# votnhan/VN_celeb_face_recognition

Hardware: AMD Instinct MI355X
Metric: embeddings/sec @ bs=256 (InceptionResnetV1, 160x160) (higher is better)
Workload: dtype bf16

## Files before the change

vn_celeb_face_recognition_amd/csrc/aux_kernels.hip:

```cpp
#include <cstdlib>
#include <algorithm>
#include "kernels.h"
#include "storage_unit.h"

namespace vnf {

typedef __bf16 bf16x8_t __attribute__((ext_vector_type(8)));
typedef _Float16 f16x8_t __attribute__((ext_vector_type(8)));
typedef float f32x4_t __attribute__((ext_vector_type(4)));

template <typename T> __device__ __forceinline__ float to_f(T v) { return (float)v; }

template <typename TI, typename TO>
__global__ void pack_input_kernel(const TI* __restrict__ x, TO* __restrict__ y, int n, int hw) {
  const size_t total = (size_t)n * hw;
  for (size_t i = blockIdx.x * (size_t)blockDim.x + threadIdx.x; i < total; i += (size_t)gridDim.x * blockDim.x) {
    const size_t img = i / hw, p = i - img * hw;
    const TI* src = x + img * 3 * (size_t)hw + p;
    if constexpr (sizeof(TO) == sizeof(pf16) && __is_same(TO, pf16)) {
      const float v[8] = {to_f(src[0]), to_f(src[hw]), to_f(src[2 * (size_t)hw]), 0.f, 0.f, 0.f, 0.f, 0.f};
      Unit<pf16>::store(y + i * 8, v);
    } else {
      TO o[8];
      o[0] = (TO)to_f(src[0]);
      o[1] = (TO)to_f(src[hw]);
      o[2] = (TO)to_f(src[2 * (size_t)hw]);
#pragma unroll
      for (int c = 3; c < 8; ++c) o[c] = (TO)0.f;
      TO* dst = y + i * 8;
      if constexpr (sizeof(TO) == 2) {
        *reinterpret_cast<uint4*>(dst) = *reinterpret_cast<const uint4*>(o);
      } else {
        *reinterpret_cast<uint4*>(dst) = *reinterpret_cast<const uint4*>(o);
        *reinterpret_cast<uint4*>(dst + 4) = *reinterpret_cast<const uint4*>(o + 4);
      }
    }
  }
}

template <typename TI>
static hipError_t pack_dispatch_out(const void* x, void* out, int dtype, int n, int hw, hipStream_t s) {
  const size_t total = (size_t)n * hw;
  const int blocks = (int)((total + 255) / 256 < 4096 ? (total + 255) / 256 : 4096);
  if (blocks == 0) return hipSuccess;
  switch (dtype) {
    case BF16: hipLaunchKernelGGL((pack_input_kernel<TI, __bf16>), dim3(blocks), dim3(256), 0, s, (const TI*)x, (__bf16*)out, n, hw); break;
    case F16: hipLaunchKernelGGL((pack_input_kernel<TI, _Float16>), dim3(blocks), dim3(256), 0, s, (const TI*)x, (_Float16*)out, n, hw); break;
    case F32: hipLaunchKernelGGL((pack_input_kernel<TI, float>), dim3(blocks), dim3(256), 0, s, (const TI*)x, (float*)out, n, hw); break;
    case F16P: hipLaunchKernelGGL((pack_input_kernel<TI, pf16>), dim3(blocks), dim3(256), 0, s, (const TI*)x, (pf16*)out, n, hw); break;
    default: return hipErrorInvalidValue;
  }
  return hipGetLastError();
}

hipError_t launch_pack_input(const void* x, int x_dtype, void* out, int dtype, int n, int hw, hipStream_t s) {
  switch (x_dtype) {
    case F32: return pack_dispatch_out<float>(x, out, dtype, n, hw, s);
    case BF16: return pack_dispatch_out<__bf16>(x, out, dtype, n, hw, s);
    case F16: return pack_dispatch_out<_Float16>(x, out, dtype, n, hw, s);
  }
  return hipErrorInvalidValue;
}

typedef float f2_t __attribute__((ext_vector_type(2)));

template <typename TI, typename TO>
__global__ void __launch_bounds__(256) stem_conv1a_kernel(const TI* __restrict__ x, TO* __restrict__ y, int ldy, int n,
                                                          const float* __restrict__ wt) {
  constexpr int S = 160, SO = 79;
  const unsigned total = (unsigned)n * SO * SO;
  const unsigned i = blockIdx.x * blockDim.x + threadIdx.x;
  if (i >= total) return;
  const unsigned img = i / (SO * SO), p = i - img * (SO * SO);
  const int oy = (int)(p / SO), ox = (int)(p - (unsigned)oy * SO);
  const TI* src = x + (size_t)img * 3 * S * S + (size_t)(2 * oy) * S + 2 * ox;
  float in[27];
#pragma unroll
  for (int c = 0; c < 3; ++c)
#pragma unroll
    for (int kh = 0; kh < 3; ++kh)
#pragma unroll
      for (int kw = 0; kw < 3; ++kw) in[(c * 3 + kh) * 3 + kw] = to_f(src[(size_t)c * S * S + kh * S + kw]);
  f2_t acc[16];
#pragma unroll
  for (int j = 0; j < 16; ++j) acc[j] = f2_t{wt[27 * 32 + 2 * j], wt[27 * 32 + 2 * j + 1]};
#pragma unroll
  for (int k = 0; k < 27; ++k) {
    const f2_t v2 = {in[k], in[k]};
#pragma unroll
    for (int j = 0; j < 16; ++j) acc[j] = __builtin_elementwise_fma(v2, f2_t{wt[k * 32 + 2 * j], wt[k * 32 + 2 * j + 1]}, acc[j]);
  }
  if constexpr (__is_same(TO, pf16)) {
#pragma unroll
    for (int u = 0; u < 4; ++u) {
      float v[8];
#pragma unroll
      for (int j = 0; j < 4; ++j) { v[2 * j] = fmaxf(acc[4 * u + j][0], 0.f); v[2 * j + 1] = fmaxf(acc[4 * u + j][1], 0.f); }
      Unit<pf16>::store(y + (size_t)i * ldy + u * 8, v);
    }
  } else {
    TO o[32];
#pragma unroll
    for (int j = 0; j < 16; ++j) { o[2 * j] = (TO)fmaxf(acc[j][0], 0.f); o[2 * j + 1] = (TO)fmaxf(acc[j][1], 0.f); }
    uint4* dst = reinterpret_cast<uint4*>(y + (size_t)i * ldy);
#pragma unroll
    for (int q = 0; q < (int)(32 * sizeof(TO) / 16); ++q) dst[q] = reinterpret_cast<const uint4*>(o)[q];
  }
}

template <typename TI, typename TO>
__global__ void __launch_bounds__(256) stem_conv1a_mfma_kernel(const TI* __restrict__ x, TO* __restrict__ y, int ldy, int n,
                                                               const float* __restrict__ wt) {
  constexpr int S = 160, SO = 79, NPX = SO * SO, G = 4;
  const int lane = threadIdx.x & 63, col = lane & 15, g = lane >> 4;
  const unsigned total = (unsigned)n * NPX;
  const unsigned ngroups = (total + 15) / 16;
  const unsigned nwaves = gridDim.x * 4, w0 = blockIdx.x * 4 + (threadIdx.x >> 6);
  float wa[2][7], bias[2][4];
  int koff[7];
#pragma unroll
  for (int t = 0; t < 7; ++t) {
    const int k = 4 * t + g;
    wa[0][t] = k < 27 ? wt[k * 32 + col] : 0.f;
    wa[1][t] = k < 27 ? wt[k * 32 + 16 + col] : 0.f;
    koff[t] = k < 27 ? (k / 9) * S * S + ((k % 9) / 3) * S + k % 3 : 0;
  }
#pragma unroll
  for (int ct = 0; ct < 2; ++ct)
#pragma unroll
    for (int e = 0; e < 4; ++e) bias[ct][e] = wt[27 * 32 + 16 * ct + 4 * g + e];
  const int cst = (g & 1) * 16 + (g >> 1) * 8;
  for (unsigned gi = w0 * G; gi < ngroups; gi += nwaves * G) {
    float xb[G][7];
#pragma unroll
    for (int q = 0; q < G; ++q) {
      const unsigned i = min((gi + q) * 16 + col, total - 1);
      const unsigned img = i / NPX, p = i - img * NPX;
      const int oy = (int)(p / SO), ox = (int)(p - (unsigned)oy * SO);
      const TI* src = x + (size_t)img * 3 * S * S + (size_t)(2 * oy) * S + 2 * ox;
#pragma unroll
      for (int t = 0; t < 7; ++t) xb[q][t] = to_f(src[koff[t]]);
    }
#pragma unroll
    for (int q = 0; q < G; ++q) {
      typedef float f4 __attribute__((ext_vector_type(4)));
      f4 a0 = {bias[0][0], bias[0][1], bias[0][2], bias[0][3]}, a1 = {bias[1][0], bias[1][1], bias[1][2], bias[1][3]};
#pragma unroll
      for (int t = 0; t < 7; ++t) {
        a0 = __builtin_amdgcn_mfma_f32_16x16x4f32(wa[0][t], xb[q][t], a0, 0, 0, 0);
        a1 = __builtin_amdgcn_mfma_f32_16x16x4f32(wa[1][t], xb[q][t], a1, 0, 0, 0);
      }
      const unsigned i = (gi + q) * 16 + col;
      const bool ok = gi + q < ngroups && i < total;
      if constexpr (__is_same(TO, pf16)) {
        typedef _Float16 h4 __attribute__((ext_vector_type(4)));
        h4 h0, l0, h1, l1;
#pragma unroll
        for (int e = 0; e < 4; ++e) {
          const sf16 s0(fmaxf(a0[e], 0.f)), s1(fmaxf(a1[e], 0.f));
          h0[e] = s0.hi; l0[e] = s0.lo;
          h1[e] = s1.hi; l1[e] = s1.lo;
        }
        const uint2 ph0 = __builtin_bit_cast(uint2, h0), ph1 = __builtin_bit_cast(uint2, h1);
        const uint2 pl0 = __builtin_bit_cast(uint2, l0), pl1 = __builtin_bit_cast(uint2, l1);
        const auto hx = __builtin_amdgcn_permlane16_swap(ph0.x, ph1.x, false, false);
        const auto hy = __builtin_amdgcn_permlane16_swap(ph0.y, ph1.y, false, false);
        const auto lx = __builtin_amdgcn_permlane16_swap(pl0.x, pl1.x, false, false);
        const auto ly = __builtin_amdgcn_permlane16_swap(pl0.y, pl1.y, false, false);
        if (ok) {
          char* d = reinterpret_cast<char*>(y) + ((size_t)i * ldy + cst) * 4;
          *reinterpret_cast<uint4*>(d) = uint4{hx[0], hy[0], hx[1], hy[1]};
          *reinterpret_cast<uint4*>(d + 16) = uint4{lx[0], ly[0], lx[1], ly[1]};
        }
      } else {
        typedef TO t4 __attribute__((ext_vector_type(4)));
        t4 o0, o1;
#pragma unroll
        for (int e = 0; e < 4; ++e) { o0[e] = (TO)fmaxf(a0[e], 0.f); o1[e] = (TO)fmaxf(a1[e], 0.f); }
        const uint2 p0 = __builtin_bit_cast(uint2, o0), p1 = __builtin_bit_cast(uint2, o1);
        const auto sx = __builtin_amdgcn_permlane16_swap(p0.x, p1.x, false, false);
        const auto sy = __builtin_amdgcn_permlane16_swap(p0.y, p1.y, false, false);
        if (ok) *reinterpret_cast<uint4*>(y + (size_t)i * ldy + cst) = uint4{sx[0], sy[0], sx[1], sy[1]};
      }
    }
  }
}

template <typename TI>
static hipError_t stem_dispatch_out(const void* x, void* y, int ldy, int dtype, int n, const float* wt, bool mfma, hipStream_t s) {
  if (mfma && n > 0 && (dtype == BF16 || dtype == F16 || dtype == F16P)) {
    const unsigned ngroups = ((unsigned)n * 79 * 79 + 15) / 16;
    const int blocks = (int)((ngroups + 15) / 16 < 2048 ? (ngroups + 15) / 16 : 2048);
    if (dtype == BF16) hipLaunchKernelGGL((stem_conv1a_mfma_kernel<TI, __bf16>), dim3(blocks), dim3(256), 0, s, (const TI*)x, (__bf16*)y, ldy, n, wt);
    else if (dtype == F16) hipLaunchKernelGGL((stem_conv1a_mfma_kernel<TI, _Float16>), dim3(blocks), dim3(256), 0, s, (const TI*)x, (_Float16*)y, ldy, n, wt);
    else hipLaunchKernelGGL((stem_conv1a_mfma_kernel<TI, pf16>), dim3(blocks), dim3(256), 0, s, (const TI*)x, (pf16*)y, ldy, n, wt);
    return hipGetLastError();
  }
  const unsigned total = (unsigned)n * 79 * 79;
  const int blocks = (int)((total + 255) / 256);
  if (blocks == 0) return hipSuccess;
  switch (dtype) {
    case BF16: hipLaunchKernelGGL((stem_conv1a_kernel<TI, __bf16>), dim3(blocks), dim3(256), 0, s, (const TI*)x, (__bf16*)y, ldy, n, wt); break;
    case F16: hipLaunchKernelGGL((stem_conv1a_kernel<TI, _Float16>), dim3(blocks), dim3(256), 0, s, (const TI*)x, (_Float16*)y, ldy, n, wt); break;
    case F32: hipLaunchKernelGGL((stem_conv1a_kernel<TI, float>), dim3(blocks), dim3(256), 0, s, (const TI*)x, (float*)y, ldy, n, wt); break;
    case F16P: hipLaunchKernelGGL((stem_conv1a_kernel<TI, pf16>), dim3(blocks), dim3(256), 0, s, (const TI*)x, (pf16*)y, ldy, n, wt); break;
    default: return hipErrorInvalidValue;
  }
  return hipGetLastError();
}

hipError_t launch_stem_conv1a(const void* x, int x_dtype, void* y, int ldy, int dtype, int n, const float* wt, bool mfma,
                              hipStream_t s) {
  switch (x_dtype) {
    case F32: return stem_dispatch_out<float>(x, y, ldy, dtype, n, wt, mfma, s);
    case BF16: return stem_dispatch_out<__bf16>(x, y, ldy, dtype, n, wt, mfma, s);
    case F16: return stem_dispatch_out<_Float16>(x, y, ldy, dtype, n, wt, mfma, s);
  }
  return hipErrorInvalidValue;
}

template <typename T, int K, int PAD, bool INSIDE>
__global__ void maxpool_kernel(const T* __restrict__ x, int ldx, T* __restrict__ y, int ldy, int n, int H, int W, int C,
                               int Ho, int Wo) {
  typedef Unit<T> U;
  constexpr int N = U::N;
  constexpr bool kCeil = !INSIDE && PAD == 0;
  constexpr int TAPS = kCeil ? 1 : K;
  const int cc = C / N;
  const unsigned total = (unsigned)n * Ho * Wo * cc;
  for (unsigned i = blockIdx.x * blockDim.x + threadIdx.x; i < total; i += gridDim.x * blockDim.x) {
    const unsigned p = i / cc;
    const int c = (int)(i - p * cc) * N;
    const unsigned q = p / Wo;
    const int wo = (int)(p - q * Wo);
    const unsigned img = q / Ho;
    const int ho = (int)(q - img * Ho);
    float m[N];
#pragma unroll
    for (int e = 0; e < N; ++e) m[e] = -INFINITY;
    if constexpr (INSIDE && sizeof(typename U::Raw) == 16) {
      const T* xi = x + ((size_t)img * H * W + (size_t)(2 * ho) * W + 2 * wo) * ldx + c;
      typename U::Raw r[K * K];
#pragma unroll
      for (int dh = 0; dh < K; ++dh)
#pragma unroll
        for (int dw = 0; dw < K; ++dw) r[dh * K + dw] = U::raw(xi + (size_t)(dh * W + dw) * ldx);
#pragma unroll
      for (int t = 0; t < K * K; ++t)
#pragma unroll
// ... 402 lines not shown
```

vn_celeb_face_recognition_amd/csrc/conv_ws.hip:

```cpp
#include <type_traits>
#include <utility>

#include "conv_device.h"
#include "stamp.h"

namespace vnf {

template <typename T, int BM, int BN, int WM, int WN, int S, int LW, bool DBG = false>
__global__ __launch_bounds__((WM* WN + LW) * 64) void conv_igemm_ws_kernel(const KArgs a) {
  extern __shared__ __attribute__((aligned(16))) char smem[];
  constexpr int ES = (int)sizeof(T);
  constexpr int CH = 16 / ES, BKE = 128 / ES;
  constexpr int WTM = BM / WM, WTN = BN / WN, TM = WTM / 16, TN = WTN / 16;
  constexpr int NC = WM * WN, NT = (NC + LW) * 64;
  constexpr int PA = BM / 8, PB = BN / 8;
  constexpr int LA = PA / LW, LB = PB / LW;
  constexpr int STAGE = (BM + BN) * 128;
  constexpr int CST = BN + 4;
  constexpr int EPI_LDS = (BM * CST * 4 <= S * STAGE && (BM * (BN / 8)) / (NC * 64) <= 8) ? S * STAGE : (BM / WM) * CST * 4;
  constexpr int EPASS = (BM * CST * 4 <= EPI_LDS) ? 1 : WM;
  static_assert(S >= 3 && PA % LW == 0 && PB % LW == 0, "pieces divide over the loader waves");

  const int tid = threadIdx.x, lane = tid & 63;
  const int wave = __builtin_amdgcn_readfirstlane(tid >> 6);
// ... 494 lines not shown
          const uint2 ph0 = __builtin_bit_cast(uint2, h0), ph1 = __builtin_bit_cast(uint2, h1);
          const uint2 pl0 = __builtin_bit_cast(uint2, l0), pl1 = __builtin_bit_cast(uint2, l1);
          const auto hx = __builtin_amdgcn_permlane16_swap(ph0.x, ph1.x, false, false);
          const auto hy = __builtin_amdgcn_permlane16_swap(ph0.y, ph1.y, false, false);
          const auto lx = __builtin_amdgcn_permlane16_swap(pl0.x, pl1.x, false, false);
          const auto ly = __builtin_amdgcn_permlane16_swap(pl0.y, pl1.y, false, false);
          if (m < a.M && c < a.Cout) {
            char* d = dcol + (size_t)m * dld * ES;
            *reinterpret_cast<uint4*>(d) = uint4{hx[0], hy[0], hx[1], hy[1]};
            *reinterpret_cast<uint4*>(d + 16) = uint4{lx[0], ly[0], lx[1], ly[1]};
          }
        } else {
          tx4 o0, o1;
#pragma unroll
          for (int e = 0; e < 4; ++e) { o0[e] = (elem_t)v0[e]; o1[e] = (elem_t)v1[e]; }
          const uint2 p0 = __builtin_bit_cast(uint2, o0), p1 = __builtin_bit_cast(uint2, o1);
          const auto sx = __builtin_amdgcn_permlane16_swap(p0.x, p1.x, false, false);
          const auto sy = __builtin_amdgcn_permlane16_swap(p0.y, p1.y, false, false);
          if (m < a.M && c < a.Cout)
            *reinterpret_cast<uint4*>(dcol + (size_t)m * dld * ES) = uint4{sx[0], sy[0], sx[1], sy[1]};
        }
      }
    }
  }
}

struct WsCfg { int bm, bn, wm, wn, s, lw; };
static constexpr WsCfg kWs[] = {
    {256, 128, 2, 2, 3, 4}, {256, 128, 4, 1, 3, 4}, {128, 128, 2, 2, 3, 4}, {128, 128, 2, 2, 4, 4},
    {256, 64, 4, 1, 3, 4},  {128, 192, 2, 2, 3, 4}, {128, 256, 2, 2, 3, 4}, {128, 64, 2, 2, 4, 4},
    {256, 128, 2, 2, 3, 2}, {128, 128, 2, 2, 4, 2}, {128, 192, 2, 2, 3, 2}, {192, 128, 2, 2, 3, 4},
    {160, 256, 2, 2, 3, 4}, {160, 192, 2, 2, 3, 4},
    {64, 64, 2, 2, 4, 4},   {64, 128, 2, 2, 4, 4},  {32, 64, 2, 2, 6, 4},   {32, 128, 2, 2, 4, 4},  {64, 64, 2, 2, 8, 4},
};
constexpr int kNumWs = (int)(sizeof(kWs) / sizeof(kWs[0]));

int ws_num_cfgs() { return kNumWs; }
bool ws_cfg_tile(int wcfg, ConvTile& t) {
  if (wcfg < 0 || wcfg >= kNumWs) return false;
  t = ConvTile{2, kWs[wcfg].bm, kWs[wcfg].bn, kWs[wcfg].wm, kWs[wcfg].wn, kWs[wcfg].s};
  return true;
}

bool ws_cfg_ok(const ConvArgs& a, int wcfg) {
  if (wcfg < 0 || wcfg >= kNumWs) return false;
  const WsCfg& c = kWs[wcfg];
  if (a.Cout <= c.bn / 2) return false;
  if (((a.Cout + c.bn - 1) / c.bn) * c.bn > a.cout_pad) return false;
  if ((c.bn % 64) && a.Cout % c.bn) return false;
  const int lds = c.s * (c.bm + c.bn) * 128 + (a.Kpad / (128 / dtype_size(a.dtype))) * 8 * 16;
  return lds <= 160 * 1024;
}

template <typename T, int BM, int BN, int WM, int WN, int S, int LW>
static hipError_t launch_one_tile(const KArgs& k, hipStream_t s) {
  allow_dynamic_lds<conv_igemm_ws_kernel<T, BM, BN, WM, WN, S, LW>>(160 * 1024);
  KArgs kk = k;
  const int lds = S * (BM + BN) * 128 + k.nkt * 8 * 16;
  const int tiles_m = (k.M + BM - 1) / BM;
  kk.tiles_n = (k.Cout + BN - 1) / BN;
  kk.nblk = tiles_m * kk.tiles_n;
  hipLaunchKernelGGL((conv_igemm_ws_kernel<T, BM, BN, WM, WN, S, LW>), dim3(kk.nblk), dim3((WM * WN + LW) * 64), lds, s,
                     kk);
  return hipGetLastError();
}

// ... 106 lines not shown
```

vn_celeb_face_recognition_amd/csrc/engine.cpp:

```cpp
#include "engine.h"
#include "split_f16.h"

#include <cstdio>
#include <cstring>

namespace vnf {

static thread_local std::string g_err;
void set_error(const std::string& msg) { g_err = msg; }
int fail(int code, const std::string& msg) {
  g_err = msg;
  return code;
}
const char* last_error_cstr() { return g_err.c_str(); }

HandleBase::~HandleBase() {
  for (void* p : allocs) (void)hipFree(p);
}
void* HandleBase::dalloc(size_t bytes) {
  void* p = nullptr;
  if (bytes == 0) bytes = 16;
  hipError_t e = hipMalloc(&p, bytes);
  if (e != hipSuccess) {
    set_error(std::string("hipMalloc: ") + hipGetErrorString(e));
// ... 220 lines not shown
      const int nn = (i1 - n0) < step ? (i1 - n0) : step;
      for (int oi = g.first; oi < g.last; ++oi) {
        if (report) {
          hipEvent_t e0;
          VNF_HIP(hipEventCreate(&e0));
          VNF_HIP(hipEventRecord(e0, s));
          prof_ev.push_back(e0);
          prof_op.push_back(oi);
        }
        if (fused_at[oi] >= 0) {
          const FusedStack& f = fused[fused_at[oi]];
          const int rc = launch_fused(f, n0, nn, s);
          if (rc != VNF_OK) return rc;
          oi = f.end() - 1;
          continue;
        }
        const Op& op = ops[oi];
        const Buf* ib = op.src >= 0 ? &bufs[op.src] : nullptr;
        switch (op.kind) {
          case Op::PACK:
            if (ex.prep_src)
              VNF_HIP(launch_emotion_prep(ex.prep_src + (size_t)n0 * ex.prep_s * ex.prep_s * 3, nn, ex.prep_s, at(op.dst, n0), dtype, true, s));
            else
              VNF_HIP(launch_pack_input((const char*)x + n0 * x_image, x_dtype, at(op.dst, n0), dtype, nn, in_size * in_size, s));
            break;
          case Op::CONV: {
            const ConvLayer& L = convs[op.layer];
            hipError_t err = launch_conv(conv_args(L, n0, nn), s);
            if (err != hipSuccess) return fail(VNF_E_HIP, L.name + ": " + hipGetErrorString(err));
            break;
          }
          case Op::STEM1:
            VNF_HIP(launch_stem_conv1a((const char*)x + n0 * x_image, x_dtype, at(op.dst, n0), bufs[op.dst].C, dtype, nn, stem_wt,
                                       env.stem1a_mfma != 0, s));
            break;
          case Op::MAXPOOL:
            VNF_HIP(launch_maxpool(at(op.src, n0), ib->C, at(op.dst, n0, op.dst_coff), bufs[op.dst].C, dtype, nn, ib->H, ib->W, ib->C,
                                   op.window, s));
            break;
          case Op::AVGPOOL:
            VNF_HIP(launch_avgpool(at(op.src, n0), ib->C, at(op.dst, n0), dtype, nn, ib->H * ib->W, ib->C, s));
            break;
          case Op::L2NORM:
            VNF_HIP(launch_l2norm(emb_raw + (size_t)n0 * 512, out + (size_t)n0 * 512, nn, 512, s));
            break;
          case Op::DWCONV: {
            if (!f32_plan) return fail(VNF_E_INVALID, "depthwise conv: fp32 / split-f16 plans only");
            const DwLayer& d = dws[op.layer];
            const Buf& xb = bufs[d.x_buf];
            VNF_HIP(launch_dwconv3x3(at_f32(d.x_buf, n0), at_f32(d.o_buf, n0), nn, xb.H, xb.W, d.C, d.stride, d.w, d.bias, d.slope,
                                     dtype == F16X2, s));
            break;
          }
          case Op::RSTEM:
            if (!f32_plan || !x) return fail(VNF_E_INVALID, "retina stem: fp32 / split-f16 plans on caller frames only");
            VNF_HIP(launch_retina_stem((const uint8_t*)x + (size_t)n0 * op.frame_h * op.frame_w * 3, nn, op.frame_h, op.frame_w, rstem_wa,
                                       rstem_bias, 0.1f, at_f32(op.dst, n0), dtype == F16X2, s));
            break;
          case Op::DWPW: {
            if (!f32_plan) return fail(VNF_E_INVALID, "dw+pw: fp32 / split-f16 plans only");
            const DwPwLayer& d = dwpws[op.layer];
            const Buf& xb = bufs[d.x_buf];
            VNF_HIP(launch_dwpw(at_f32(d.x_buf, n0), at_f32(d.o_buf, n0), nn, xb.H, xb.W, d.cin, d.cout, d.stride, d.dw, d.dbias, d.slope,
                                d.pw, d.pbias, d.slope, dtype == F16X2, s));
            break;
          }
          case Op::UPADD: {
// ... 102 lines not shown
```

vn_celeb_face_recognition_amd/csrc/engine.h:

```cpp
#pragma once
#include <hip/hip_runtime.h>
#include <stdint.h>

#include <string>
#include <unordered_map>
#include <vector>

#include "../../include/vnface.h"
#include "kernels.h"

namespace vnf {

void set_error(const std::string& msg);
int fail(int code, const std::string& msg);
const char* last_error_cstr();

#define VNF_HIP(expr)                                                                         \
  do {                                                                                        \
    hipError_t _e = (expr);                                                                   \
    if (_e != hipSuccess)                                                                     \
      return ::vnf::fail(VNF_E_HIP, std::string(#expr) + ": " + hipGetErrorString(_e));       \
  } while (0)

enum class HandleKind { Encoder = 1, Mlp, Mtcnn, MlpTrainer, Retina, HeadTrainer, ConvProbe };
// ... 97 lines not shown
  float slope = 0.f;
  std::string name;
};

struct SeLayer {
  std::string name;
  int C, part_buf;
  float *w1 = nullptr, *b1 = nullptr, *w2 = nullptr, *b2 = nullptr;
  float slope_se = 0.f, slope_out = 0.f;
};

struct Group { int first, last, chunk; };

struct FusedStack {
  enum class Kind { StemMid, Block35, Block17 } kind = Kind::Block17;
  int first = 0, last = 0;
  int in_buf = -1, out_buf = -1;
  int nblocks = 0;
  int conv0 = 0;
  void* wstream = nullptr;
  float* bias = nullptr;
  void* wtail = nullptr;
  bool active = false;
  bool stack = false;
  double macs_alg = 0;
  int ext_last = 0, ext_conv = -1, ext_out_buf = -1;
  bool ext = false;
  int end() const { return ext ? ext_last : last; }
};

struct Tap { int buf, coff, C; };

struct EncoderEnv {
  int fuse = 31, direct_stem = 1, stem1a_mfma = 1, retina_fuse = 3, ws_persist = 1;
  int stem_chunk = 0, ir100_chunk1 = 0, ir100_chunk2 = 0;
  int autotune = 1, force_cfg = -2, tune_lanes = 0, autotune_log = 0;
  bool tune_final = true;
  std::string tune_cache;
  static EncoderEnv read();
};

struct RunExtra {
  float* out2 = nullptr;
  const uint8_t* prep_src = nullptr;
  int prep_s = 0;
};

constexpr int ARCH_MLP = -1, ARCH_RNET = -2, ARCH_ONET = -3, ARCH_RETINA = -5;

struct Encoder : HandleBase {
  static constexpr HandleKind KIND = HandleKind::Encoder;
  Encoder() : HandleBase(KIND) {}
  ~Encoder() override;
  int arch, dtype, max_batch, in_size;
  std::vector<Buf> bufs;
  std::vector<ConvLayer> convs;
  std::vector<DwLayer> dws;
  std::vector<DwPwLayer> dwpws;
  std::vector<SeLayer> ses;
  float *rstem_wa = nullptr, *rstem_bias = nullptr;
  std::vector<Op> ops;
  std::vector<Group> groups;
  std::vector<FusedStack> fused;
  std::vector<int> fused_at;
  int prepare_fused();
  int launch_fused(const FusedStack& f, int n0, int nn, hipStream_t s);
  std::unordered_map<std::string, Tap> taps;
// ... 52 lines not shown
```

vn_celeb_face_recognition_amd/csrc/kernels.h:

```cpp
#pragma once
#include <hip/hip_runtime.h>
#include <stdint.h>

#include "../../include/vnface.h"

namespace vnf {

enum DType { F32 = 0, BF16 = 1, F16 = 2, F16X2 = 5, F16P = 6 };
inline int dtype_size(int dt) { return (dt == F32 || dt == F16X2 || dt == F16P) ? 4 : 2; }
inline int dtype_chan_align(int dt) { return dt == F16P ? 8 : 16 / dtype_size(dt); }

enum Act { ACT_NONE = 0, ACT_RELU = 1, ACT_PRELU = 2 };

struct ConvSeg {
  int c0, c1;
  void* ptr;
  int ld;
};

struct ConvArgs {
  int dtype;
  const void* x;
  int ldx;
  int H, W, Cin;
  int Ho, Wo;
  int KH, KW, sh, sw, ph, pw;
  const void* w;
  int K, Kpad;
  const float* bias;
  int ncls;
  int cout_pad;
  const int4* ktab;
  int M, Cout;
  int nseg;
  ConvSeg seg[4];
  const void* res;
  int ldres;
  int act;
  const float* slope;
  int out_f32;
  int cfg;
  int ws_persist;
};

hipError_t launch_conv(const ConvArgs& a, hipStream_t s);
int conv_num_cfgs();
bool conv_cfg_ok(const ConvArgs& a, int cfg);
void conv_family_sizes(int sizes[3]);
struct ConvTile { int family, bm, bn, wm, wn, stages; };
bool conv_cfg_tile(int cfg, ConvTile& t);

hipError_t launch_pack_input(const void* x, int x_dtype, void* out, int dtype, int n, int hw, hipStream_t s);

hipError_t launch_stem_conv1a(const void* x, int x_dtype, void* y, int ldy, int dtype, int n, const float* wt, bool mfma,
                              hipStream_t s);

struct PoolWindow { int k, pad; bool ceil; };
inline int pool_out_size(int in, PoolWindow w) {
  const int span = in + 2 * w.pad - w.k;
  return span < 0 && !w.ceil ? 0 : (span + (w.ceil ? 1 : 0)) / 2 + 1;
}
hipError_t launch_maxpool(const void* x, int ldx, void* y, int ldy, int dtype, int n, int H, int W, int C, PoolWindow w,
                          hipStream_t s);

hipError_t launch_emotion_prep(const uint8_t* faces, int n, int S, void* out, int out_dtype, bool packed, hipStream_t s);

hipError_t launch_augment_faces(const uint8_t* faces, int n_faces, int S, const int32_t* index, const vnf_aug_param* params, int n,
                                int T, void* x_out, int out_dtype, uint8_t* u8_out, hipStream_t s);

hipError_t launch_softmax_topk(const float* logits, int n, int C, int k, int32_t* idx, float* prob, hipStream_t s);

hipError_t launch_copy_rows_f32(const float* src, int lds, float* dst, int ldd, int n, int C, hipStream_t s);

hipError_t launch_avgpool(const void* x, int ldx, void* y, int dtype, int n, int HW, int C, hipStream_t s);

struct SeWeights { const float *w1, *b1, *w2, *b2; float slope_se, slope_out; };
int se_slices(int dtype, int HW, int C);
hipError_t launch_se_block(const void* t, const void* res, void* y, int dtype, int n, int HW, int C, const SeWeights& w, float* part,
                           size_t part_stride, hipStream_t s);

hipError_t launch_l2norm(const float* x, float* y, int n, int C, hipStream_t s);

hipError_t launch_head_eval(const float* logits, int ld, int C, int n, const int64_t* target, float* logp, int32_t* amax,
                            float* prob, float* nll, int32_t* hit, float* sums, hipStream_t s);

hipError_t launch_dwconv3x3(const float* x, float* y, int n, int H, int W, int C, int stride, const float* w9c,
                            const float* bias, float slope, bool split, hipStream_t s);
// ... 13 lines not shown
```

Baseline: 269,700.

## Stage stem conv input row bands in LDS for MFMA conv1a

The MFMA stem conv kernel now gives each block one image and a band of 8 output rows. It copies the band's input rows for all three channels into shared memory, using vectorized 16-byte loads when the input is aligned, then runs the MFMA per 16-pixel tile reading from LDS. This replaces strided, overlapping global gathers per output pixel with a coalesced staging load and reuse of overlapping stride-2 windows. In exchange it adds a block barrier, LDS use, and a fixed grid of n*10 blocks with partially idle waves on the last band.

```diff
diff --git a/vn_celeb_face_recognition_amd/csrc/aux_kernels.hip b/vn_celeb_face_recognition_amd/csrc/aux_kernels.hip
--- a/vn_celeb_face_recognition_amd/csrc/aux_kernels.hip
+++ b/vn_celeb_face_recognition_amd/csrc/aux_kernels.hip
@@ -1,6 +1,7 @@
 #include <cstdlib>
 #include <algorithm>
 #include "kernels.h"
+#include "stem1a_row.h"
 #include "storage_unit.h"
 
 namespace vnf {
@@ -63,6 +64,7 @@
 }
 
 typedef float f2_t __attribute__((ext_vector_type(2)));
+constexpr int kStem1aBand = 8;
 
 template <typename TI, typename TO>
 __global__ void __launch_bounds__(256) stem_conv1a_kernel(const TI* __restrict__ x, TO* __restrict__ y, int ldy, int n,
@@ -111,77 +113,56 @@
 template <typename TI, typename TO>
 __global__ void __launch_bounds__(256) stem_conv1a_mfma_kernel(const TI* __restrict__ x, TO* __restrict__ y, int ldy, int n,
                                                                const float* __restrict__ wt) {
-  constexpr int S = 160, SO = 79, NPX = SO * SO, G = 4;
-  const int lane = threadIdx.x & 63, col = lane & 15, g = lane >> 4;
-  const unsigned total = (unsigned)n * NPX;
-  const unsigned ngroups = (total + 15) / 16;
-  const unsigned nwaves = gridDim.x * 4, w0 = blockIdx.x * 4 + (threadIdx.x >> 6);
-  float wa[2][7], bias[2][4];
-  int koff[7];
-#pragma unroll
-  for (int t = 0; t < 7; ++t) {
-    const int k = 4 * t + g;
-    wa[0][t] = k < 27 ? wt[k * 32 + col] : 0.f;
-    wa[1][t] = k < 27 ? wt[k * 32 + 16 + col] : 0.f;
-    koff[t] = k < 27 ? (k / 9) * S * S + ((k % 9) / 3) * S + k % 3 : 0;
-  }
-#pragma unroll
-  for (int ct = 0; ct < 2; ++ct)
-#pragma unroll
-    for (int e = 0; e < 4; ++e) bias[ct][e] = wt[27 * 32 + 16 * ct + 4 * g + e];
-  const int cst = (g & 1) * 16 + (g >> 1) * 8;
-  for (unsigned gi = w0 * G; gi < ngroups; gi += nwaves * G) {
-    float xb[G][7];
-#pragma unroll
-    for (int q = 0; q < G; ++q) {
-      const unsigned i = min((gi + q) * 16 + col, total - 1);
-      const unsigned img = i / NPX, p = i - img * NPX;
-      const int oy = (int)(p / SO), ox = (int)(p - (unsigned)oy * SO);
-      const TI* src = x + (size_t)img * 3 * S * S + (size_t)(2 * oy) * S + 2 * ox;
-#pragma unroll
-      for (int t = 0; t < 7; ++t) xb[q][t] = to_f(src[koff[t]]);
-    }
-#pragma unroll
-    for (int q = 0; q < G; ++q) {
-      typedef float f4 __attribute__((ext_vector_type(4)));
-      f4 a0 = {bias[0][0], bias[0][1], bias[0][2], bias[0][3]}, a1 = {bias[1][0], bias[1][1], bias[1][2], bias[1][3]};
-#pragma unroll
-      for (int t = 0; t < 7; ++t) {
-        a0 = __builtin_amdgcn_mfma_f32_16x16x4f32(wa[0][t], xb[q][t], a0, 0, 0, 0);
-        a1 = __builtin_amdgcn_mfma_f32_16x16x4f32(wa[1][t], xb[q][t], a1, 0, 0, 0);
-      }
-      const unsigned i = (gi + q) * 16 + col;
-      const bool ok = gi + q < ngroups && i < total;
-      if constexpr (__is_same(TO, pf16)) {
-        typedef _Float16 h4 __attribute__((ext_vector_type(4)));
-        h4 h0, l0, h1, l1;
-#pragma unroll
-        for (int e = 0; e < 4; ++e) {
-          const sf16 s0(fmaxf(a0[e], 0.f)), s1(fmaxf(a1[e], 0.f));
-          h0[e] = s0.hi; l0[e] = s0.lo;
-          h1[e] = s1.hi; l1[e] = s1.lo;
+  typedef Stem1aRow<TI> P;
+  constexpr int S = P::S, SO = P::SO, R = kStem1aBand, BANDS = (SO + R - 1) / R;
+  constexpr int ROWB = S * (int)sizeof(TI), CS = (2 * R + 1) * ROWB;
+  __shared__ __attribute__((aligned(16))) char smem[3 * CS];
+  const int tid = threadIdx.x, lane = tid & 63, wave = tid >> 6;
+  const int img = blockIdx.x / BANDS, oy0 = (blockIdx.x - img * BANDS) * R;
+  const int nrow = min(R, SO - oy0);
+  const int span = (2 * nrow + 1) * ROWB;
+  const char* src = reinterpret_cast<const char*>(x) + ((size_t)img * 3 * S + 2 * oy0) * ROWB;
+  if ((reinterpret_cast<uintptr_t>(x) & 15) == 0) {
+    const int per = span / 16;
+    for (int i = tid; i < 3 * per; i += 256) {
+      const int c = i / per, o = (i - c * per) * 16;
+      *reinterpret_cast<uint4*>(smem + c * CS + o) = *reinterpret_cast<const uint4*>(src + (size_t)c * S * ROWB + o);
+    }
+  } else {
+    const int per = span / (int)sizeof(TI);
+    for (int i = tid; i < 3 * per; i += 256) {
+      const int c = i / per, o = i - c * per;
+      reinterpret_cast<TI*>(smem + c * CS)[o] = reinterpret_cast<const TI*>(src + (size_t)c * S * ROWB)[o];
+    }
+  }
+  P prod;
+  prod.init(wt, lane, CS, ROWB);
+  __syncthreads();
+  const int ntile = nrow * P::TILES;
+  for (int j = wave; j < ntile; j += 8) {
+    float xb[2][7];
+    int row[2], tile[2];
+#pragma unroll
+    for (int q = 0; q < 2; ++q) {
+      const int jj = min(j + 4 * q, ntile - 1);
+      row[q] = jj / P::TILES;
+      tile[q] = jj - row[q] * P::TILES;
+      prod.fetch(smem, 2 * row[q] * ROWB, (2 * row[q] + 2) * ROWB, tile[q], xb[q]);
+    }
+#pragma unroll
+    for (int q = 0; q < 2; ++q) {
+      const bool live = j + 4 * q < ntile;
+      const size_t i0 = (size_t)img * SO * SO + (size_t)(oy0 + row[q]) * SO;
+      prod.template compute<TO>(xb[q], tile[q], [&](int px, int c0, const uint4& v0, const uint4& v1) {
+        if (!live || px >= SO) return;
+        if constexpr (__is_same(TO, pf16)) {
+          char* d = reinterpret_cast<char*>(y) + ((i0 + px) * ldy + c0) * 4;
+          *reinterpret_cast<uint4*>(d) = v0;
+          *reinterpret_cast<uint4*>(d + 16) = v1;
+        } else {
+          *reinterpret_cast<uint4*>(y + (i0 + px) * ldy + c0) = v0;
         }
-        const uint2 ph0 = __builtin_bit_cast(uint2, h0), ph1 = __builtin_bit_cast(uint2, h1);
-        const uint2 pl0 = __builtin_bit_cast(uint2, l0), pl1 = __builtin_bit_cast(uint2, l1);
-        const auto hx = __builtin_amdgcn_permlane16_swap(ph0.x, ph1.x, false, false);
-        const auto hy = __builtin_amdgcn_permlane16_swap(ph0.y, ph1.y, false, false);
-        const auto lx = __builtin_amdgcn_permlane16_swap(pl0.x, pl1.x, false, false);
-        const auto ly = __builtin_amdgcn_permlane16_swap(pl0.y, pl1.y, false, false);
-        if (ok) {
-          char* d = reinterpret_cast<char*>(y) + ((size_t)i * ldy + cst) * 4;
-          *reinterpret_cast<uint4*>(d) = uint4{hx[0], hy[0], hx[1], hy[1]};
-          *reinterpret_cast<uint4*>(d + 16) = uint4{lx[0], ly[0], lx[1], ly[1]};
-        }
-      } else {
-        typedef TO t4 __attribute__((ext_vector_type(4)));
-        t4 o0, o1;
-#pragma unroll
-        for (int e = 0; e < 4; ++e) { o0[e] = (TO)fmaxf(a0[e], 0.f); o1[e] = (TO)fmaxf(a1[e], 0.f); }
-        const uint2 p0 = __builtin_bit_cast(uint2, o0), p1 = __builtin_bit_cast(uint2, o1);
-        const auto sx = __builtin_amdgcn_permlane16_swap(p0.x, p1.x, false, false);
-        const auto sy = __builtin_amdgcn_permlane16_swap(p0.y, p1.y, false, false);
-        if (ok) *reinterpret_cast<uint4*>(y + (size_t)i * ldy + cst) = uint4{sx[0], sy[0], sx[1], sy[1]};
-      }
+      });
     }
   }
 }
@@ -189,8 +170,7 @@
 template <typename TI>
 static hipError_t stem_dispatch_out(const void* x, void* y, int ldy, int dtype, int n, const float* wt, bool mfma, hipStream_t s) {
   if (mfma && n > 0 && (dtype == BF16 || dtype == F16 || dtype == F16P)) {
-    const unsigned ngroups = ((unsigned)n * 79 * 79 + 15) / 16;
-    const int blocks = (int)((ngroups + 15) / 16 < 2048 ? (ngroups + 15) / 16 : 2048);
+    const int blocks = n * ((79 + kStem1aBand - 1) / kStem1aBand);
     if (dtype == BF16) hipLaunchKernelGGL((stem_conv1a_mfma_kernel<TI, __bf16>), dim3(blocks), dim3(256), 0, s, (const TI*)x, (__bf16*)y, ldy, n, wt);
     else if (dtype == F16) hipLaunchKernelGGL((stem_conv1a_mfma_kernel<TI, _Float16>), dim3(blocks), dim3(256), 0, s, (const TI*)x, (_Float16*)y, ldy, n, wt);
     else hipLaunchKernelGGL((stem_conv1a_mfma_kernel<TI, pf16>), dim3(blocks), dim3(256), 0, s, (const TI*)x, (pf16*)y, ldy, n, wt);
diff --git a/vn_celeb_face_recognition_amd/csrc/stem1a_row.h b/vn_celeb_face_recognition_amd/csrc/stem1a_row.h
--- /dev/null
+++ b/vn_celeb_face_recognition_amd/csrc/stem1a_row.h
@@ -0,0 +1,84 @@
+#pragma once
+#include <hip/hip_runtime.h>
+
+#include "split_f16.h"
+
+namespace vnf {
+
+template <typename TI>
+struct Stem1aRow {
+  static constexpr int S = 160, SO = 79, TILES = 5;
+  float wa[2][7], bias[2][4];
+  int off[7];
+  int third;
+  int col, cst;
+
+  __device__ __forceinline__ void init(const float* __restrict__ wt, int lane, int ch_stride, int row_stride) {
+    col = lane & 15;
+    third = 0;
+    const int g = lane >> 4;
+#pragma unroll
+    for (int t = 0; t < 7; ++t) {
+      const int k = 4 * t + g;
+      wa[0][t] = k < 27 ? wt[k * 32 + col] : 0.f;
+      wa[1][t] = k < 27 ? wt[k * 32 + 16 + col] : 0.f;
+      const int kh = k < 27 ? (k % 9) / 3 : 0;
+      off[t] = k < 27 ? (k / 9) * ch_stride + (kh == 1 ? row_stride : 0) + (k % 3) * (int)sizeof(TI) : 0;
+      third |= (kh == 2) << t;
+    }
+#pragma unroll
+    for (int ct = 0; ct < 2; ++ct)
+#pragma unroll
+      for (int e = 0; e < 4; ++e) bias[ct][e] = wt[27 * 32 + 16 * ct + 4 * g + e];
+    cst = (g & 1) * 16 + (g >> 1) * 8;
+  }
+
+  __device__ __forceinline__ void fetch(const char* smem, int r0, int r2, int tile, float (&xb)[7]) const {
+    const int xo = 2 * min(16 * tile + col, SO - 1) * (int)sizeof(TI);
+    const int x0 = r0 + xo, x2 = r2 + xo;
+#pragma unroll
+    for (int t = 0; t < 7; ++t)
+      xb[t] = (float)*reinterpret_cast<const TI*>(smem + ((third >> t) & 1 ? x2 : x0) + off[t]);
+  }
+
+  template <typename TO, typename Store>
+  __device__ __forceinline__ void compute(const float (&xb)[7], int tile, Store&& store) const {
+    typedef float f4 __attribute__((ext_vector_type(4)));
+    f4 a0 = {bias[0][0], bias[0][1], bias[0][2], bias[0][3]}, a1 = {bias[1][0], bias[1][1], bias[1][2], bias[1][3]};
+#pragma unroll
+    for (int t = 0; t < 7; ++t) {
+      a0 = __builtin_amdgcn_mfma_f32_16x16x4f32(wa[0][t], xb[t], a0, 0, 0, 0);
+      a1 = __builtin_amdgcn_mfma_f32_16x16x4f32(wa[1][t], xb[t], a1, 0, 0, 0);
+    }
+    const int px = 16 * tile + col;
+    if constexpr (__is_same(TO, pf16)) {
+      typedef _Float16 h4 __attribute__((ext_vector_type(4)));
+      h4 h0, l0, h1, l1;
+#pragma unroll
+      for (int e = 0; e < 4; ++e) {
+        const sf16 s0(fmaxf(a0[e], 0.f)), s1(fmaxf(a1[e], 0.f));
+        h0[e] = s0.hi; l0[e] = s0.lo;
+        h1[e] = s1.hi; l1[e] = s1.lo;
+      }
+      const uint2 ph0 = __builtin_bit_cast(uint2, h0), ph1 = __builtin_bit_cast(uint2, h1);
+      const uint2 pl0 = __builtin_bit_cast(uint2, l0), pl1 = __builtin_bit_cast(uint2, l1);
+      const auto hx = __builtin_amdgcn_permlane16_swap(ph0.x, ph1.x, false, false);
+      const auto hy = __builtin_amdgcn_permlane16_swap(ph0.y, ph1.y, false, false);
+      const auto lx = __builtin_amdgcn_permlane16_swap(pl0.x, pl1.x, false, false);
+      const auto ly = __builtin_amdgcn_permlane16_swap(pl0.y, pl1.y, false, false);
+      store(px, cst, uint4{hx[0], hy[0], hx[1], hy[1]}, uint4{lx[0], ly[0], lx[1], ly[1]});
+    } else {
+      typedef TO t4 __attribute__((ext_vector_type(4)));
+      t4 o0, o1;
+#pragma unroll
+      for (int e = 0; e < 4; ++e) { o0[e] = (TO)fmaxf(a0[e], 0.f); o1[e] = (TO)fmaxf(a1[e], 0.f); }
+      const uint2 p0 = __builtin_bit_cast(uint2, o0), p1 = __builtin_bit_cast(uint2, o1);
+      const auto sx = __builtin_amdgcn_permlane16_swap(p0.x, p1.x, false, false);
+      const auto sy = __builtin_amdgcn_permlane16_swap(p0.y, p1.y, false, false);
+      const uint4 v = {sx[0], sy[0], sx[1], sy[1]};
+      store(px, cst, v, v);
+    }
+  }
+};
+
+}
```

Result: no change. 270,400, median of 3 (+0.3%).

## Stage stem conv input bands in shared memory with per-image row-band blocks

Applied to the files above, without the earlier changes.

The MFMA stem conv kernel now assigns each block one image and an 8-output-row band. The block loads the needed input rows for all three channels into LDS using 16-byte vector loads, and waves then read the 3x3 stride-2 taps from shared memory. Tap loads for the next 16-pixel group are prefetched while the current MFMAs run. This replaces scattered per-pixel global gathers, which re-fetched overlapping input, at the cost of LDS occupancy, a barrier, and a new 16-byte alignment requirement on the input pointer (unaligned inputs fall back to the scalar kernel).

```diff
diff --git a/vn_celeb_face_recognition_amd/csrc/aux_kernels.hip b/vn_celeb_face_recognition_amd/csrc/aux_kernels.hip
--- a/vn_celeb_face_recognition_amd/csrc/aux_kernels.hip
+++ b/vn_celeb_face_recognition_amd/csrc/aux_kernels.hip
@@ -108,14 +108,47 @@
   }
 }
 
+
+template <typename TI> __device__ __forceinline__ unsigned tap_bits(const TI* p) {
+  if constexpr (sizeof(TI) == 2) return *reinterpret_cast<const unsigned short*>(p);
+  else return *reinterpret_cast<const unsigned*>(p);
+}
+template <typename TI> __device__ __forceinline__ float tap_value(unsigned b) {
+  if constexpr (sizeof(TI) == 2) return to_f(__builtin_bit_cast(TI, (unsigned short)b));
+  else return __builtin_bit_cast(float, b);
+}
+
+constexpr int kStemBand = 8, kStemBands = (79 + kStemBand - 1) / kStemBand;
+
 template <typename TI, typename TO>
-__global__ void __launch_bounds__(256) stem_conv1a_mfma_kernel(const TI* __restrict__ x, TO* __restrict__ y, int ldy, int n,
-                                                               const float* __restrict__ wt) {
-  constexpr int S = 160, SO = 79, NPX = SO * SO, G = 4;
-  const int lane = threadIdx.x & 63, col = lane & 15, g = lane >> 4;
-  const unsigned total = (unsigned)n * NPX;
-  const unsigned ngroups = (total + 15) / 16;
-  const unsigned nwaves = gridDim.x * 4, w0 = blockIdx.x * 4 + (threadIdx.x >> 6);
+__global__ void __launch_bounds__(256, sizeof(TI) == 4 ? 5 : 6)
+stem_conv1a_mfma_kernel(const TI* __restrict__ x, TO* __restrict__ y, int ldy, int n, const float* __restrict__ wt) {
+  constexpr int S = 160, SO = 79, BR = kStemBand, NB = kStemBands, RI = 2 * BR + 1, PL = RI * S;
+  constexpr int EPC = 16 / (int)sizeof(TI);
+  constexpr int NL = (3 * PL / EPC + 255) / 256;
+  constexpr int NG = (SO + 15) / 16;
+  static_assert(BR % 4 == 0 && S % EPC == 0 && (2 * BR * S) % EPC == 0, "band rows start on a 16-byte boundary");
+  __shared__ __attribute__((aligned(16))) TI sm[3 * PL];
+  const int tid = threadIdx.x, lane = tid & 63, col = lane & 15, g = lane >> 4;
+  const int img = blockIdx.x / NB, band = blockIdx.x - img * NB;
+  const int rows_in = min(RI, S - 2 * BR * band), rows_out = min(BR, SO - BR * band);
+  {
+    const int nchunk = rows_in * (S / EPC);
+    const TI* src = x + (size_t)img * 3 * S * S + (size_t)(2 * BR * band) * S;
+    typedef unsigned u4 __attribute__((ext_vector_type(4)));
+    u4 st[NL];
+#pragma unroll
+    for (int m = 0; m < NL; ++m) {
+      const int idx = tid + 256 * m, c = (idx >= nchunk) + (idx >= 2 * nchunk), r = idx - c * nchunk;
+      st[m] = u4{0u, 0u, 0u, 0u};
+      if (idx < 3 * nchunk) st[m] = *reinterpret_cast<const u4*>(src + (size_t)c * S * S + r * EPC);
+    }
+#pragma unroll
+    for (int m = 0; m < NL; ++m) {
+      const int idx = tid + 256 * m, c = (idx >= nchunk) + (idx >= 2 * nchunk), r = idx - c * nchunk;
+      if (idx < 3 * nchunk) *reinterpret_cast<u4*>(sm + c * PL + r * EPC) = st[m];
+    }
+  }
   float wa[2][7], bias[2][4];
   int koff[7];
 #pragma unroll
@@ -123,35 +156,41 @@
     const int k = 4 * t + g;
     wa[0][t] = k < 27 ? wt[k * 32 + col] : 0.f;
     wa[1][t] = k < 27 ? wt[k * 32 + 16 + col] : 0.f;
-    koff[t] = k < 27 ? (k / 9) * S * S + ((k % 9) / 3) * S + k % 3 : 0;
+    koff[t] = k < 27 ? (k / 9) * PL + ((k % 9) / 3) * S + k % 3 : 0;
   }
 #pragma unroll
   for (int ct = 0; ct < 2; ++ct)
 #pragma unroll
     for (int e = 0; e < 4; ++e) bias[ct][e] = wt[27 * 32 + 16 * ct + 4 * g + e];
   const int cst = (g & 1) * 16 + (g >> 1) * 8;
-  for (unsigned gi = w0 * G; gi < ngroups; gi += nwaves * G) {
-    float xb[G][7];
-#pragma unroll
-    for (int q = 0; q < G; ++q) {
-      const unsigned i = min((gi + q) * 16 + col, total - 1);
-      const unsigned img = i / NPX, p = i - img * NPX;
-      const int oy = (int)(p / SO), ox = (int)(p - (unsigned)oy * SO);
-      const TI* src = x + (size_t)img * 3 * S * S + (size_t)(2 * oy) * S + 2 * ox;
-#pragma unroll
-      for (int t = 0; t < 7; ++t) xb[q][t] = to_f(src[koff[t]]);
-    }
-#pragma unroll
-    for (int q = 0; q < G; ++q) {
+  __syncthreads();
+  for (int rr = 0; rr < BR / 4; ++rr) {
+    const int ry = (tid >> 6) * (BR / 4) + rr;
+    if (ry >= rows_out) break;
+    const TI* rowp = sm + 2 * ry * S;
+    const size_t i0 = ((size_t)img * SO + (BR * band + ry)) * SO;
+    auto taps = [&](unsigned (&v)[7], int q) {
+      const int ox = min(16 * q + col, SO - 1);
+#pragma unroll
+      for (int t = 0; t < 7; ++t) v[t] = tap_bits(rowp + 2 * ox + koff[t]);
+    };
+    float xb[7];
+    unsigned xn[7];
+    taps(xn, 0);
+#pragma unroll 1
+    for (int q = 0; q < NG; ++q) {
+#pragma unroll
+      for (int t = 0; t < 7; ++t) xb[t] = tap_value<TI>(xn[t]);
+      taps(xn, min(q + 1, NG - 1));
       typedef float f4 __attribute__((ext_vector_type(4)));
       f4 a0 = {bias[0][0], bias[0][1], bias[0][2], bias[0][3]}, a1 = {bias[1][0], bias[1][1], bias[1][2], bias[1][3]};
 #pragma unroll
       for (int t = 0; t < 7; ++t) {
-        a0 = __builtin_amdgcn_mfma_f32_16x16x4f32(wa[0][t], xb[q][t], a0, 0, 0, 0);
-        a1 = __builtin_amdgcn_mfma_f32_16x16x4f32(wa[1][t], xb[q][t], a1, 0, 0, 0);
-      }
-      const unsigned i = (gi + q) * 16 + col;
-      const bool ok = gi + q < ngroups && i < total;
+        a0 = __builtin_amdgcn_mfma_f32_16x16x4f32(wa[0][t], xb[t], a0, 0, 0, 0);
+        a1 = __builtin_amdgcn_mfma_f32_16x16x4f32(wa[1][t], xb[t], a1, 0, 0, 0);
+      }
+      const bool ok = 16 * q + col < SO;
+      const size_t i = i0 + 16 * q + col;
       if constexpr (__is_same(TO, pf16)) {
         typedef _Float16 h4 __attribute__((ext_vector_type(4)));
         h4 h0, l0, h1, l1;
@@ -188,9 +227,8 @@
 
 template <typename TI>
 static hipError_t stem_dispatch_out(const void* x, void* y, int ldy, int dtype, int n, const float* wt, bool mfma, hipStream_t s) {
-  if (mfma && n > 0 && (dtype == BF16 || dtype == F16 || dtype == F16P)) {
-    const unsigned ngroups = ((unsigned)n * 79 * 79 + 15) / 16;
-    const int blocks = (int)((ngroups + 15) / 16 < 2048 ? (ngroups + 15) / 16 : 2048);
+  if (mfma && n > 0 && (dtype == BF16 || dtype == F16 || dtype == F16P) && reinterpret_cast<uintptr_t>(x) % 16 == 0) {
+    const int blocks = n * kStemBands;
     if (dtype == BF16) hipLaunchKernelGGL((stem_conv1a_mfma_kernel<TI, __bf16>), dim3(blocks), dim3(256), 0, s, (const TI*)x, (__bf16*)y, ldy, n, wt);
     else if (dtype == F16) hipLaunchKernelGGL((stem_conv1a_mfma_kernel<TI, _Float16>), dim3(blocks), dim3(256), 0, s, (const TI*)x, (_Float16*)y, ldy, n, wt);
     else hipLaunchKernelGGL((stem_conv1a_mfma_kernel<TI, pf16>), dim3(blocks), dim3(256), 0, s, (const TI*)x, (pf16*)y, ldy, n, wt);
```

After: 259,400 before, 261,800 after, median of 6. No clear change (+0.9%).

## Add row-band stem conv1a kernel with LDS-staged, double-buffered input reuse

Applied to the files above, without the earlier changes.

Adds a persistent stem conv1a kernel in which each block takes a band of 4 output rows. The block stages the 9 needed input rows of all 3 channels into LDS with double buffering and register prefetch of the next band. Each wave then computes one output row with fp32 MFMA, reading the overlapping 3x3 stride-2 windows from LDS instead of re-fetching them from global memory. The new kernel becomes the default (mode 2) and needs 16-byte input alignment. A new 224x192 warp-specialized conv tile config is also added to the autotune candidates.

```diff
diff --git a/vn_celeb_face_recognition_amd/csrc/aux_kernels.hip b/vn_celeb_face_recognition_amd/csrc/aux_kernels.hip
--- a/vn_celeb_face_recognition_amd/csrc/aux_kernels.hip
+++ b/vn_celeb_face_recognition_amd/csrc/aux_kernels.hip
@@ -1,5 +1,6 @@
 #include <cstdlib>
 #include <algorithm>
+#include <type_traits>
 #include "kernels.h"
 #include "storage_unit.h"
 
@@ -186,9 +187,150 @@
   }
 }
 
+struct Stem1aRows { static constexpr int R = 4, NB = (79 + R - 1) / R; };
+
+template <typename TI, typename TO>
+__global__ void __launch_bounds__(256) stem_conv1a_rows_kernel(const TI* __restrict__ x, TO* __restrict__ y, int ldy, int n,
+                                                               const float* __restrict__ wt) {
+  constexpr int S = 160, SO = 79, NPX = SO * SO, R = Stem1aRows::R, NB = Stem1aRows::NB, ES = (int)sizeof(TI);
+  static_assert(R == 4, "one output row per wave");
+  constexpr int RI = 2 * R + 1, CS = RI * S;
+  constexpr int RC = S * ES / 16, CSC = CS * ES / 16;
+  constexpr int NLD = (3 * RI * RC + 255) / 256;
+  constexpr int BUFB = 3 * CS * ES + 16;
+  typedef unsigned u4 __attribute__((ext_vector_type(4)));
+  typedef float f4 __attribute__((ext_vector_type(4)));
+  __shared__ __attribute__((aligned(16))) char sm[2 * BUFB];
+  const int tid = threadIdx.x, lane = tid & 63, col = lane & 15, g = lane >> 4;
+  const int wave = __builtin_amdgcn_readfirstlane(tid >> 6);
+  const int nbands = n * NB;
+  u4 v[NLD];
+  auto fetch = [&](int b) {
+    const int img = b / NB, oy0 = (b - img * NB) * R;
+    const int cpc = (2 * min(R, SO - oy0) + 1) * RC;
+    const u4* src = reinterpret_cast<const u4*>(x + (size_t)img * 3 * S * S + (size_t)(2 * oy0) * S);
+#pragma unroll
+    for (int j = 0; j < NLD; ++j) {
+      const int q = min(tid + j * 256, 3 * cpc - 1);
+      const int c = (q >= cpc) + (q >= 2 * cpc);
+      v[j] = src[c * (S * S * ES / 16) + q - c * cpc];
+    }
+  };
+  auto stash = [&](int b, int buf) {
+    const int oy0 = (b % NB) * R;
+    const int cpc = (2 * min(R, SO - oy0) + 1) * RC;
+#pragma unroll
+    for (int j = 0; j < NLD; ++j) {
+      const int q = tid + j * 256;
+      const int c = (q >= cpc) + (q >= 2 * cpc);
+      if (q < 3 * cpc) reinterpret_cast<u4*>(sm + buf * BUFB)[c * CSC + q - c * cpc] = v[j];
+    }
+  };
+  int band = blockIdx.x;
+  if (band >= nbands) return;
+  float wa[2][7], bias[2][4];
+  int la[7];
+#pragma unroll
+  for (int t = 0; t < 7; ++t) {
+    const int k = 4 * t + g;
+    wa[0][t] = k < 27 ? wt[k * 32 + col] : 0.f;
+    wa[1][t] = k < 27 ? wt[k * 32 + 16 + col] : 0.f;
+    la[t] = (2 * wave * S + 2 * col + (k < 27 ? (k / 9) * CS + ((k % 9) / 3) * S + k % 3 : 0)) * ES;
+  }
+#pragma unroll
+  for (int ct = 0; ct < 2; ++ct)
+#pragma unroll
+    for (int e = 0; e < 4; ++e) bias[ct][e] = wt[27 * 32 + 16 * ct + 4 * g + e];
+  const int cst = (g & 1) * 16 + (g >> 1) * 8;
+  fetch(band);
+  stash(band, 0);
+  __builtin_amdgcn_s_waitcnt(0x0f70);
+
+  auto groups = [&](auto buf_c, auto j0_c, auto nj_c, unsigned row0) {
+    constexpr int BUF = decltype(buf_c)::value, J0 = decltype(j0_c)::value, NJ = decltype(nj_c)::value;
+    float xb[NJ][7];
+#pragma unroll
+    for (int j = 0; j < NJ; ++j)
+#pragma unroll
+      for (int t = 0; t < 7; ++t)
+        xb[j][t] = to_f(*reinterpret_cast<const TI*>(sm + la[t] + (BUF * BUFB + (J0 + j) * 32 * ES)));
+    f4 a0[NJ], a1[NJ];
+#pragma unroll
+    for (int j = 0; j < NJ; ++j) {
+      a0[j] = f4{bias[0][0], bias[0][1], bias[0][2], bias[0][3]};
+      a1[j] = f4{bias[1][0], bias[1][1], bias[1][2], bias[1][3]};
+    }
+#pragma unroll
+    for (int t = 0; t < 7; ++t)
+#pragma unroll
+      for (int j = 0; j < NJ; ++j) {
+        a0[j] = __builtin_amdgcn_mfma_f32_16x16x4f32(wa[0][t], xb[j][t], a0[j], 0, 0, 0);
+        a1[j] = __builtin_amdgcn_mfma_f32_16x16x4f32(wa[1][t], xb[j][t], a1[j], 0, 0, 0);
+      }
+#pragma unroll
+    for (int j = 0; j < NJ; ++j) {
+      const unsigned i = row0 + (J0 + j) * 16 + col;
+      const bool ok = (J0 + j + 1) * 16 <= SO || col < SO - (J0 + j) * 16;
+      if constexpr (__is_same(TO, pf16)) {
+        typedef _Float16 h4 __attribute__((ext_vector_type(4)));
+        h4 h0, l0, h1, l1;
+#pragma unroll
+        for (int e = 0; e < 4; ++e) {
+          const sf16 s0(fmaxf(a0[j][e], 0.f)), s1(fmaxf(a1[j][e], 0.f));
+          h0[e] = s0.hi; l0[e] = s0.lo;
+          h1[e] = s1.hi; l1[e] = s1.lo;
+        }
+        const uint2 ph0 = __builtin_bit_cast(uint2, h0), ph1 = __builtin_bit_cast(uint2, h1);
+        const uint2 pl0 = __builtin_bit_cast(uint2, l0), pl1 = __builtin_bit_cast(uint2, l1);
+        const auto hx = __builtin_amdgcn_permlane16_swap(ph0.x, ph1.x, false, false);
+        const auto hy = __builtin_amdgcn_permlane16_swap(ph0.y, ph1.y, false, false);
+        const auto lx = __builtin_amdgcn_permlane16_swap(pl0.x, pl1.x, false, false);
+        const auto ly = __builtin_amdgcn_permlane16_swap(pl0.y, pl1.y, false, false);
+        if (ok) {
+          char* d = reinterpret_cast<char*>(y) + ((size_t)i * ldy + cst) * 4;
+          *reinterpret_cast<uint4*>(d) = uint4{hx[0], hy[0], hx[1], hy[1]};
+          *reinterpret_cast<uint4*>(d + 16) = uint4{lx[0], ly[0], lx[1], ly[1]};
+        }
+      } else {
+        typedef TO t4 __attribute__((ext_vector_type(4)));
+        t4 o0, o1;
+#pragma unroll
+        for (int e = 0; e < 4; ++e) { o0[e] = (TO)fmaxf(a0[j][e], 0.f); o1[e] = (TO)fmaxf(a1[j][e], 0.f); }
+        const uint2 p0 = __builtin_bit_cast(uint2, o0), p1 = __builtin_bit_cast(uint2, o1);
+        const auto sx = __builtin_amdgcn_permlane16_swap(p0.x, p1.x, false, false);
+        const auto sy = __builtin_amdgcn_permlane16_swap(p0.y, p1.y, false, false);
+        if (ok) *reinterpret_cast<uint4*>(y + (size_t)i * ldy + cst) = uint4{sx[0], sy[0], sx[1], sy[1]};
+      }
+    }
+  };
+  auto one_band = [&](auto buf_c) {
+    constexpr int BUF = decltype(buf_c)::value;
+    const int next = band + gridDim.x;
+    if (next < nbands) fetch(next);
+    __syncthreads();
+    const int img = band / NB, oy0 = (band - img * NB) * R;
+    if (wave < min(R, SO - oy0)) {
+      const unsigned row0 = (unsigned)img * NPX + (unsigned)((oy0 + wave) * SO);
+      groups(buf_c, std::integral_constant<int, 0>{}, std::integral_constant<int, 3>{}, row0);
+      groups(buf_c, std::integral_constant<int, 3>{}, std::integral_constant<int, 2>{}, row0);
+    }
+    if (next < nbands) stash(next, BUF ^ 1);
+    band = next;
+    return next < nbands;
+  };
+  while (one_band(std::integral_constant<int, 0>{}) && one_band(std::integral_constant<int, 1>{})) {}
+}
+
 template <typename TI>
-static hipError_t stem_dispatch_out(const void* x, void* y, int ldy, int dtype, int n, const float* wt, bool mfma, hipStream_t s) {
-  if (mfma && n > 0 && (dtype == BF16 || dtype == F16 || dtype == F16P)) {
+static hipError_t stem_dispatch_out(const void* x, void* y, int ldy, int dtype, int n, const float* wt, int mode, hipStream_t s) {
+  if (mode >= 2 && n > 0 && (dtype == BF16 || dtype == F16 || dtype == F16P) && ((uintptr_t)x & 15) == 0) {
+    const int blocks = std::min(n * Stem1aRows::NB, 1024);
+    if (dtype == BF16) hipLaunchKernelGGL((stem_conv1a_rows_kernel<TI, __bf16>), dim3(blocks), dim3(256), 0, s, (const TI*)x, (__bf16*)y, ldy, n, wt);
+    else if (dtype == F16) hipLaunchKernelGGL((stem_conv1a_rows_kernel<TI, _Float16>), dim3(blocks), dim3(256), 0, s, (const TI*)x, (_Float16*)y, ldy, n, wt);
+    else hipLaunchKernelGGL((stem_conv1a_rows_kernel<TI, pf16>), dim3(blocks), dim3(256), 0, s, (const TI*)x, (pf16*)y, ldy, n, wt);
+    return hipGetLastError();
+  }
+  if (mode != 0 && n > 0 && (dtype == BF16 || dtype == F16 || dtype == F16P)) {
     const unsigned ngroups = ((unsigned)n * 79 * 79 + 15) / 16;
     const int blocks = (int)((ngroups + 15) / 16 < 2048 ? (ngroups + 15) / 16 : 2048);
     if (dtype == BF16) hipLaunchKernelGGL((stem_conv1a_mfma_kernel<TI, __bf16>), dim3(blocks), dim3(256), 0, s, (const TI*)x, (__bf16*)y, ldy, n, wt);
@@ -209,12 +351,12 @@
   return hipGetLastError();
 }
 
-hipError_t launch_stem_conv1a(const void* x, int x_dtype, void* y, int ldy, int dtype, int n, const float* wt, bool mfma,
+hipError_t launch_stem_conv1a(const void* x, int x_dtype, void* y, int ldy, int dtype, int n, const float* wt, int mode,
                               hipStream_t s) {
   switch (x_dtype) {
-    case F32: return stem_dispatch_out<float>(x, y, ldy, dtype, n, wt, mfma, s);
-    case BF16: return stem_dispatch_out<__bf16>(x, y, ldy, dtype, n, wt, mfma, s);
-    case F16: return stem_dispatch_out<_Float16>(x, y, ldy, dtype, n, wt, mfma, s);
+    case F32: return stem_dispatch_out<float>(x, y, ldy, dtype, n, wt, mode, s);
+    case BF16: return stem_dispatch_out<__bf16>(x, y, ldy, dtype, n, wt, mode, s);
+    case F16: return stem_dispatch_out<_Float16>(x, y, ldy, dtype, n, wt, mode, s);
   }
   return hipErrorInvalidValue;
 }
diff --git a/vn_celeb_face_recognition_amd/csrc/conv_ws.hip b/vn_celeb_face_recognition_amd/csrc/conv_ws.hip
--- a/vn_celeb_face_recognition_amd/csrc/conv_ws.hip
+++ b/vn_celeb_face_recognition_amd/csrc/conv_ws.hip
@@ -550,6 +550,7 @@
     {256, 128, 2, 2, 3, 2}, {128, 128, 2, 2, 4, 2}, {128, 192, 2, 2, 3, 2}, {192, 128, 2, 2, 3, 4},
     {160, 256, 2, 2, 3, 4}, {160, 192, 2, 2, 3, 4},
     {64, 64, 2, 2, 4, 4},   {64, 128, 2, 2, 4, 4},  {32, 64, 2, 2, 6, 4},   {32, 128, 2, 2, 4, 4},  {64, 64, 2, 2, 8, 4},
+    {224, 192, 2, 2, 3, 4},
 };
 constexpr int kNumWs = (int)(sizeof(kWs) / sizeof(kWs[0]));
 
diff --git a/vn_celeb_face_recognition_amd/csrc/engine.cpp b/vn_celeb_face_recognition_amd/csrc/engine.cpp
--- a/vn_celeb_face_recognition_amd/csrc/engine.cpp
+++ b/vn_celeb_face_recognition_amd/csrc/engine.cpp
@@ -276,7 +276,7 @@
           }
           case Op::STEM1:
             VNF_HIP(launch_stem_conv1a((const char*)x + n0 * x_image, x_dtype, at(op.dst, n0), bufs[op.dst].C, dtype, nn, stem_wt,
-                                       env.stem1a_mfma != 0, s));
+                                       env.stem1a_mfma, s));
             break;
           case Op::MAXPOOL:
             VNF_HIP(launch_maxpool(at(op.src, n0), ib->C, at(op.dst, n0, op.dst_coff), bufs[op.dst].C, dtype, nn, ib->H, ib->W, ib->C,
diff --git a/vn_celeb_face_recognition_amd/csrc/engine.h b/vn_celeb_face_recognition_amd/csrc/engine.h
--- a/vn_celeb_face_recognition_amd/csrc/engine.h
+++ b/vn_celeb_face_recognition_amd/csrc/engine.h
@@ -153,7 +153,7 @@
 struct Tap { int buf, coff, C; };
 
 struct EncoderEnv {
-  int fuse = 31, direct_stem = 1, stem1a_mfma = 1, retina_fuse = 3, ws_persist = 1;
+  int fuse = 31, direct_stem = 1, stem1a_mfma = 2, retina_fuse = 3, ws_persist = 1;
   int stem_chunk = 0, ir100_chunk1 = 0, ir100_chunk2 = 0;
   int autotune = 1, force_cfg = -2, tune_lanes = 0, autotune_log = 0;
   bool tune_final = true;
diff --git a/vn_celeb_face_recognition_amd/csrc/kernels.h b/vn_celeb_face_recognition_amd/csrc/kernels.h
--- a/vn_celeb_face_recognition_amd/csrc/kernels.h
+++ b/vn_celeb_face_recognition_amd/csrc/kernels.h
@@ -52,7 +52,7 @@
 
 hipError_t launch_pack_input(const void* x, int x_dtype, void* out, int dtype, int n, int hw, hipStream_t s);
 
-hipError_t launch_stem_conv1a(const void* x, int x_dtype, void* y, int ldy, int dtype, int n, const float* wt, bool mfma,
+hipError_t launch_stem_conv1a(const void* x, int x_dtype, void* y, int ldy, int dtype, int n, const float* wt, int mode,
                               hipStream_t s);
 
 struct PoolWindow { int k, pad; bool ceil; };
```

Result: faster. 271,000 before, 273,900 after (median of 6 runs) (+1.1%).
